# alvgaona/heart-sounds-segmentation

Hardware: AMD Instinct MI355X
Metric: PCG windows/sec FSST (1 kHz, 2000-sample) (higher is better)
Workload: dtype f32

## Files before the change

heart_sounds_segmentation_amd/csrc/fsst_canon128.hpp:

```cpp
#pragma once
#include "fsst_mfma128.hpp"

namespace hssfsst {

using h8 = _Float16 __attribute__((ext_vector_type(8)));
using u2 = unsigned __attribute__((ext_vector_type(2)));
using u4 = unsigned __attribute__((ext_vector_type(4)));
using lds_u2 = __attribute__((address_space(3))) u2;
using lds_u4 = __attribute__((address_space(3))) u4;

#define HSS_RARE_VMEM_DONE() __builtin_amdgcn_s_waitcnt(0x0f70)
constexpr int kCanonTileFrames = 64;
constexpr int kCanonRecs = 192;
constexpr int kCanonErrMul = 4;
constexpr int kCanonFlagWords = 8;
constexpr int kCanonTieWords = 32;

template <int KLO, int KC>
struct CanonCfg {
    static_assert(KC % 2 == 0 && KC >= 2 && KC <= 24 && KLO >= 0 && KLO + KC <= 32, "even band of <= 24 rows inside rows 0..31");
    static constexpr int NWIN = 128;
    static constexpr int KHI = KLO + KC - 1;
    static constexpr int H0 = KLO / 4, H1 = KHI / 4;
    static constexpr int COV0 = 4 * H0, COVN = 4 * (H1 - H0 + 1);
    static constexpr int LD = odd_up(COVN + 1), LDF = plane_ldf(KC), KOFF = KLO - COV0;
    static constexpr bool stored(int s, int half) { return 2 * s + half >= H0 && 2 * s + half <= H1; }
    static constexpr int need_row(int row)
    {
        int best = NWIN;
        for (int k = KLO; k <= KHI; ++k)
            for (int tw = 0; tw < 2; ++tw) {
                const int r = tw ? (NWIN - k) % NWIN : k;
                int d = row > r ? row - r : r - row;
                if (NWIN - d < d) d = NWIN - d;
                if (d < best) best = d;
            }
        return best;
    }
    static constexpr int need(int s, int half)
    {
        int best = NWIN;
        for (int r = 0; r < 4; ++r) {
            const int d = need_row(8 * s + 4 * half + r);
            if (d < best) best = d;
        }
        return best;
    }
    static constexpr float thr(int s, int half)
    {
        const int nd = need(s, half);
        return (nd <= 1 ? 0.5f : static_cast<float>(nd) - 0.5f) - static_cast<float>(1 + (nd <= 1 ? 0 : nd)) * kTieMargin;
    }
    static_assert(KLO >= 1, "row 0 is its own twin: acc_source / canon_put want the band above it");
    static constexpr int wave_floats() { return 2 * kCanonRecs + 2 * 16 * LD + kCanonFlagWords + kCanonTieWords; }
};


constexpr float kOffsetErr2 = 0.0625f;
struct CanonTile {
    float R2s;
    float inv;
    float r2s;
    float mean_s;
    __device__ __forceinline__ float eoff() const { return mean_s != 0.0f ? kOffsetErr2 : 0.0f; }
};

constexpr int kCanonYcGroup = 33;
constexpr int kCanonYcFrame = 4 * kCanonYcGroup * 2;
constexpr int kCanonYcRight = 80;
constexpr int kCanonZcFloats = kCanonYcFrame + 4 * 32 * 64 * 2 + 4 * 32 * kCanonYcRight * 2;
constexpr float kMeanTheta = 0.5f;

template <bool OFFS = true>
__device__ __forceinline__ CanonTile canon_land(const float (&sreg)[3], u2* xrec, float r2scale_s, float inv_c, int lane, int t0, int n)
{
    float e2 = 0.0f, s1 = 0.0f;
#pragma unroll
    for (int k = 0; k < 3; ++k) { e2 = fmaf(sreg[k], sreg[k], e2); s1 += sreg[k]; }
    const int inside = min(t0 + 128, n) - max(t0 - 64, 0);
    TileEnergy te = tile_energy(e2, s1, 0.0f);
    te.C = static_cast<float>(max(inside, 0));
    te.dcdom = te.E > 0.0f && te.S1 * te.S1 >= kDcTheta * te.C * te.E;
    auto stage = [&](const float (&x)[3], float Es, float E, float mean) -> CanonTile {
        const int eb = static_cast<int>((__float_as_uint(Es) >> 23) & 0xffu);
        const int hb = (eb - 127 + 2) >> 1;
        const int se = (eb == 0 || eb == 255) ? 127 : 127 + 14 - hb;
        const float sx = __uint_as_float(static_cast<unsigned>(se) << 23);
        CanonTile t;
        t.inv = __uint_as_float(static_cast<unsigned>(254 - se) << 23) * inv_c;
        t.R2s = r2scale_s * (E * sx) * sx;
        t.r2s = r2scale_s;
        t.mean_s = mean * sx;
#pragma unroll
        for (int k = 0; k < 3; ++k) {
            const float v = x[k] * sx;
            const _Float16 x1 = static_cast<_Float16>(v);
            const _Float16 x2 = static_cast<_Float16>(v - static_cast<float>(x1));
            const unsigned b1 = __builtin_bit_cast(unsigned short, x1), b2 = __builtin_bit_cast(unsigned short, x2);
            xrec[lane + 64 * k] = u2{b1 | (b1 << 16), b2 | (b2 << 16)};
        }
        wave_sync();
        return t;
    };
    if (__builtin_expect(te.E > 0.0f && te.S1 * te.S1 >= kMeanTheta * te.C * te.E, 0)) {
        if constexpr (!OFFS) { CanonTile r{}; r.mean_s = __builtin_nanf(""); return r; }
        const float mean = te.S1 / te.C;
        float x[3], ea = 0.0f;
#pragma unroll
        for (int k = 0; k < 3; ++k) {
            const int gi = t0 + lane + 64 * k - 64;
            x[k] = (gi >= 0 && gi < n) ? sreg[k] - mean : 0.0f;
            ea = fmaf(x[k], x[k], ea);
        }
        const float E = __int_as_float(__builtin_amdgcn_readfirstlane(__float_as_int(piece_sums(ea, 0.0f, 0.0f, 0.0f))));
        return stage(x, (E > 0.0f) ? E : te.S1 * mean, E, mean);
    }
    return stage(sreg, te.E, te.E, 0.0f);
}

struct CanonMove { int row; bool tie; };
__device__ __forceinline__ CanonMove canon_decide(int kpi, float num, float den, float R2, float eoff)
{
    constexpr int NWIN = 128;
    float shift = num * __builtin_amdgcn_rcpf(den);
    if (!(fabsf(shift) <= 1.0e6f)) shift = 0.0f;
    const float a = static_cast<float>(kpi) + shift;
    float fr = a - floorf(a) - 0.5f;
    const float s1 = 1.0f + fabsf(shift);
    asm volatile("" : "+v"(fr));
    CanonMove m;
    m.tie = fr * fr * den < (kTieErr2 * kCanonErrMul) * s1 * s1 * fmaf(eoff, den, R2) && den > kTieFloor2 * R2;
    const float r = truncf(a + copysignf(0.5f, a));
    m.row = static_cast<int>(r) & (NWIN - 1);
    return m;
}
template <int KLO, int KC, int S>
__device__ __forceinline__ bool canon_put(f2* row0, int kpi, int row, f2 V)
{
    constexpr int NWIN = 128;
    int t = row;
    float vy = V.y;
    if (!(static_cast<unsigned>(row - KLO) < static_cast<unsigned>(KC))) {
        if (!(row > NWIN / 2 && kpi != 0)) return false;
        t = NWIN - row; vy = -V.y;
        if (!(static_cast<unsigned>(t - KLO) < static_cast<unsigned>(KC))) return false;
    }
    if (S < 3 && (t >> 3) > S) return true;
    float* q = reinterpret_cast<float*>(row0 + t);
    __hip_atomic_fetch_add(q, V.x, __ATOMIC_RELAXED, __HIP_MEMORY_SCOPE_WORKGROUP);
    __hip_atomic_fetch_add(q + 1, vy, __ATOMIC_RELAXED, __HIP_MEMORY_SCOPE_WORKGROUP);
    return false;
}

template <int KLO, int KC, int TAPB = 4, bool OFFS = true, class XSig = const float*>
__device__ __forceinline__ void canon_group(const u2* xrec, const float* atab, f2* own_base, int* flag, int* tq,
                                            const double* wtab, const double* twtab, const CanonTile& tile, f2 tiny, int lane_o,
                                            XSig xsig, int n, int tg, const float* zc)
{
// ... 555 lines not shown
```

heart_sounds_segmentation_amd/csrc/fsst_launch_shape.hpp:

```cpp
#pragma once

#include <algorithm>
#include <cstddef>
#include <cstdint>
#include <vector>

namespace hssfsst {

constexpr int kMaxLdsBytes = 160 * 1024;
constexpr int kFpw128 = 64;
constexpr int kPartFloats = 8;

struct Core128Regions {
    int g0[3];
    int gpc[3];
    int npc[3];
};

inline Core128Regions core128_regions(int ngroups, long long nsig = -1)
{
    Core128Regions r{};
    const int tail2 = ngroups >= 32 ? 6 : 0;
    const int tail4 = ngroups >= 32 ? 16 : 0;
    if (ngroups < 32) {
// ... 84 lines not shown
    int rq = 0;
    bool fast = false;
    bool stripes03 = false;
    size_t lds_fixed = 0, lds_per_wave = 0;
};
constexpr MfmaFacts mfma_facts(int nwin, int klo, int K, bool stack)
{
    MfmaFacts f;
    f.fast = stack && (K & 1) == 0 && K <= 24;
    if (!mfma_length(nwin)) return f;
    const int nt = mfma_taps(nwin), rq = nwin / nt, min_waves = (nwin == 512) ? 2 : 4;
    const size_t fixed = (core128_atab_floats(rq, nt) + kCtlFloats) * sizeof(float);
    const size_t per_wave = static_cast<size_t>(wave_lds_floats(kFpw128, klo, K, rq, nt)) * sizeof(float);
    if (fixed + min_waves * per_wave > static_cast<size_t>(kMaxLdsBytes)) return f;
    f.nt = nt; f.rq = rq; f.lds_fixed = fixed; f.lds_per_wave = per_wave;
    f.stripes03 = own_s0(klo, rq) == 0 && own_s1(klo, K, rq) == 3;
    return f;
}
constexpr size_t core128_lds_bytes(const MfmaFacts& f, int wpb, bool pair)
{
    const size_t regions = pair ? wpb / 2 : wpb;
    return f.lds_fixed + regions * (f.lds_per_wave + (pair ? kPairFloats * sizeof(float) : 0));
}

struct Core128PlainRow { int nt, rq; bool fast; int wpb, s1c; bool pair; };
constexpr Core128PlainRow kCore128Plain[] = {
    {16, 8, true, 16, 3, false}, {16, 8, true, 16, -1, false},
    {16, 8, false, 16, -1, false}, {16, 8, false, 8, -1, false}, {16, 8, false, 4, -1, false},
    {16, 16, true, 8, -1, false}, {16, 16, false, 8, 3, false}, {16, 16, false, 8, -1, false},
    {16, 16, false, 4, -1, false}, {16, 16, true, 4, -1, false},
    {32, 16, true, 8, -1, true}, {32, 16, false, 8, -1, true}, {32, 16, false, 6, -1, true}, {32, 16, false, 4, -1, true},
    {32, 16, true, 8, -1, false}, {32, 16, false, 8, -1, false}, {32, 16, false, 6, -1, false}, {32, 16, true, 4, -1, false},
    {32, 16, false, 4, -1, false}, {32, 16, false, 3, -1, false}, {32, 16, false, 2, -1, false}, {32, 16, true, 2, -1, false},
};
constexpr int kCore128PlainRows = static_cast<int>(sizeof(kCore128Plain) / sizeof(kCore128Plain[0]));
constexpr int core128_plain_row(const MfmaFacts& f, bool no_pair)
{
    for (int i = 0; i < kCore128PlainRows; ++i) {
        const Core128PlainRow& r = kCore128Plain[i];
        if (r.nt == f.nt && r.rq == f.rq && r.fast == f.fast && (r.s1c < 0 || f.stripes03) && !(r.pair && no_pair)
            && core128_lds_bytes(f, r.wpb, r.pair) <= static_cast<size_t>(kMaxLdsBytes))
            return i;
    }
    return -1;
}

constexpr bool fused_rounds_full(int64_t batch, int64_t grid)
{
    const int64_t rounds = (batch + grid - 1) / grid;
    return !(batch < grid || rounds * grid * 100 > batch * 112);
}

constexpr int kT16MaxCpc = 8;
struct Team16Geometry {
    bool ok = false;
    int T = 0;
    int cpc_shift = 0;
    int nteams = 0, grid = 0;
    int slots = 0;
};
constexpr Team16Geometry team16_geometry(int G, int64_t batch, long long xstride, int cus, int WPB, int DEPTH, int pslots, int ms)
{
    Team16Geometry g;
    if (G < 1 || G > kFusedMaxGroups) return g;
    int T = 1;
    while ((WPB / 2) * T < G) T *= 2;
    if (T > cus || T > 64) return g;
    int cpc = 1, cpc_shift = 0;
    while (cpc * T < G) { cpc *= 2; ++cpc_shift; }
    if (cpc > WPB || cpc > kT16MaxCpc || G / T < 1) return g;
    if (cpc < 4 && T > 1) return g;
    int nteams = cus / T;
    if (batch < nteams) nteams = static_cast<int>(batch);
    if ((batch + nteams - 1) / nteams > 65535) return g;
    if (xstride < 1 || xstride > 0x7fffffffLL || batch > 0x7fffffffLL) return g;
    const int held_pos = WPB * (DEPTH + 3);
    const int lead = (held_pos + G / T - 1) / (G / T) + 1;
    int slots = 8;
    while (slots < 2 * lead + 2) slots *= 2;
    if (slots > ms) return g;
    if (lead + 1 > pslots) return g;
    g.ok = true; g.T = T; g.cpc_shift = cpc_shift; g.nteams = nteams; g.grid = nteams * T; g.slots = slots;
    return g;
}

struct ZscoreShape {
    int64_t grid;
    int slices;
    bool fused;
};
constexpr ZscoreShape zscore_shape(int64_t batch)
{
    int64_t zgrid = 4096;
    int slices = 1;
    if (batch < 1024) {
        slices = static_cast<int>(1024 / batch);
        if (slices > 32) slices = 32;
    }
    if (zgrid > batch * slices) zgrid = batch * slices;
    const bool fused = slices == 1 && zgrid == batch && batch >= 512;
    return {zgrid, slices, fused};
}

struct DftShape {
    int G;
    int waves;
    long long nitems;
    long long blocks;
};
constexpr DftShape dft_shape(int nk4, int K, int ncols, int64_t batch)
{
    int G = 1, best_waves = -1;
    for (int cand = 4; cand >= 1; cand >>= 1) {
        const size_t pw = static_cast<size_t>(dft_wave_lds_floats(nk4, K, cand)) * sizeof(float);
        int w = static_cast<int>(static_cast<size_t>(kMaxLdsBytes) / pw);
        if (w > 8) w = 8;
        if (w < 1) continue;
        int per_cu = static_cast<int>(static_cast<size_t>(kMaxLdsBytes) / (pw * w)) * w;
        if (per_cu > 32) per_cu = 32;
        if (per_cu >= 16) { G = cand; best_waves = per_cu; break; }
        if (per_cu > best_waves) { G = cand; best_waves = per_cu; }
    }
    if (ncols <= 16) G = 1;
    const size_t per_wave = static_cast<size_t>(dft_wave_lds_floats(nk4, K, G)) * sizeof(float);
    int waves = static_cast<int>(static_cast<size_t>(kMaxLdsBytes) / per_wave);
    if (waves > 8) waves = 8;
    if (waves < 1) return {G, 0, 0, 0};
    const int ntiles = (ncols + 16 * G - 1) / (16 * G);
    const long long nitems = static_cast<long long>(batch) * ntiles;
    long long blocks = (nitems + waves - 1) / waves;
    if (blocks > 256 * 64) blocks = 256 * 64;
    return {G, waves, nitems, blocks};
}

}
// ... 1 lines not shown
```

heart_sounds_segmentation_amd/csrc/fsst_team16.hpp:

```cpp
#pragma once
#include "fsst_mfma128.hpp"
#include "fsst_canon128.hpp"

namespace hssfsst {

using gu64 = __attribute__((address_space(1))) unsigned long long;

constexpr int kT16PartFloats = 6;
constexpr int kT16BlockWords = 8;
constexpr int kT16MaxBlocks = kFusedMaxGroups / kStatBlock;
constexpr int kT16SlotWords = kT16MaxBlocks * kT16BlockWords;
constexpr int kT16MaxSlots = 64;
constexpr int kT16StatFloats = 12;
constexpr int t16_ctl_base(int slots) { return 16 + 64 + 192 + 2 * slots + kT16StatFloats * slots; }
constexpr int t16_ctl_floats(int pslots, int slots) { return t16_ctl_base(slots) + pslots * (kT16MaxCpc * kT16PartFloats + 2); }
template <int KLO, int KC>
constexpr int t16_room() { return 160 * 1024 / 4 - kCanonLdsTabFloats - 16 * CanonCfg<KLO, KC>::wave_floats(); }
template <int KLO, int KC>
constexpr int t16_slots() { return t16_room<KLO, KC>() >= t16_ctl_floats(16, kT16MaxSlots) ? kT16MaxSlots : kT16MaxSlots / 2; }
template <int KLO, int KC>
constexpr int t16_pslots()
{
    constexpr int room = t16_room<KLO, KC>(), sl = t16_slots<KLO, KC>();
    return room >= t16_ctl_floats(32, sl) ? 32 : room >= t16_ctl_floats(16, sl) ? 16 : 0;
}

struct Team16Params {
    const float* x;
    float* out;
    const float* atab;
    const double* wtab;
    const double* twtab;
    unsigned long long* mail;
    unsigned* status;
    float r2scale_s;
    float inv_c;
    int n, nsig, col0, ncols;
    long long xstride;
    int team;
    int cpc_shift;
    int slots;
    unsigned seq;
    unsigned spin_ticks;
    unsigned* arrive;
    unsigned arrive_base;
    unsigned* abort_word;
    unsigned* fallbacks;
    unsigned launch;
    unsigned* done;
    unsigned done_base;
    unsigned* host_done;
    double inv_total, inv_total1;
};


constexpr int kT16HeldBase = 104;
#define HSS_T16_PAIRS(X) X(0, 104, 105) X(1, 106, 107) X(2, 108, 109) X(3, 110, 111) X(4, 112, 113) X(5, 114, 115) \
                         X(6, 116, 117) X(7, 118, 119) X(8, 120, 121) X(9, 122, 123) X(10, 124, 125) X(11, 126, 127)
template <int P>
__device__ __forceinline__ void held_put(f2 a, f2 b)
{
#define HSS_T16_PUT(N, LO, HI) if constexpr (P == N) asm volatile("v_pk_mul_f32 v[" #LO ":" #HI "], %0, %1" :: "v"(a), "v"(b) : "v" #LO, "v" #HI);
    HSS_T16_PAIRS(HSS_T16_PUT)
#undef HSS_T16_PUT
}
template <int P>
__device__ __forceinline__ f2 held_zscore(f2 m)
{
    f2 d, e;
#define HSS_T16_ZS(N, LO, HI) if constexpr (P == N) asm volatile("v_pk_add_f32 %0, v[" #LO ":" #HI "], %1 op_sel:[0,0] op_sel_hi:[1,0] neg_lo:[0,1] neg_hi:[0,1]" : "=v"(d) : "v"(m));
    HSS_T16_PAIRS(HSS_T16_ZS)
#undef HSS_T16_ZS
    asm("v_pk_mul_f32 %0, %1, %2 op_sel:[0,1] op_sel_hi:[1,1]" : "=v"(e) : "v"(d), "v"(m));
    return e;
}

template <class OT>
__device__ __forceinline__ void team16_store4(char* dst, f2 lo, f2 hi)
{
    static_assert(sizeof(OT) == 2, "2-byte output elements");
    using o2 = OT __attribute__((ext_vector_type(2)));
    using w2 = unsigned __attribute__((ext_vector_type(2)));
    const w2 w = {__builtin_bit_cast(unsigned, __builtin_convertvector(lo, o2)), __builtin_bit_cast(unsigned, __builtin_convertvector(hi, o2))};
    __builtin_nontemporal_store(w, reinterpret_cast<w2*>(dst));
}

template <int KLO, int KC, int WPB, int DEPTH, class OT = float>
__global__ __launch_bounds__(64 * WPB, WPB / 4) __attribute__((amdgpu_num_vgpr(52))) void fsst_team16_kernel(Team16Params p)
{
    constexpr int OB = static_cast<int>(sizeof(OT));
    using C = CanonCfg<KLO, KC>;
    static_assert(WPB % 4 == 0 && DEPTH >= 1 && DEPTH <= 2, "whole waves per SIMD; two held groups (v104 .. v127)");
    static_assert(DEPTH == 2, "the kernel is compiled for 104 allocatable registers + 24 fixed ones");
    constexpr int K = KC, ATAB = kCanonLdsTabFloats;
    extern __shared__ __attribute__((aligned(16))) float smem[];
    const int n = p.n;
    const int lane = threadIdx.x & 63;
    const int wv = __builtin_amdgcn_readfirstlane(threadIdx.x >> 6);
    float* atab = smem;
    int* next_q = reinterpret_cast<int*>(smem + ATAB);
    unsigned* dead = reinterpret_cast<unsigned*>(smem + ATAB) + 1;
    unsigned* cls_lds = reinterpret_cast<unsigned*>(smem + ATAB + 16);
    unsigned* ppk_lds = reinterpret_cast<unsigned*>(smem + ATAB + 80);
    unsigned* ready = reinterpret_cast<unsigned*>(smem + ATAB + 272);
    constexpr int MS = t16_slots<KLO, KC>(), PSLOTS = t16_pslots<KLO, KC>();
    unsigned* claim = ready + MS;
    float4* fin = reinterpret_cast<float4*>(smem + ATAB + 272 + 2 * MS);
    static_assert(PSLOTS >= 16, "the CU's own partials need LDS beside the wave regions");
    float* part_lds = smem + ATAB + t16_ctl_base(MS);
    int* pcnt_lds = reinterpret_cast<int*>(part_lds + PSLOTS * kT16MaxCpc * kT16PartFloats);
    float* wbase = smem + ATAB + t16_ctl_floats(PSLOTS, MS) + wv * C::wave_floats();
    u2* xrec = reinterpret_cast<u2*>(wbase);
    f2* own_base = reinterpret_cast<f2*>(wbase + 2 * kCanonRecs);
    int* flag = reinterpret_cast<int*>(own_base + 16 * C::LD);
    int* tq = flag + kCanonFlagWords;

    unsigned arrived = 0u;
    if (threadIdx.x == 64) arrived = __hip_atomic_fetch_add(p.arrive, 1u, __ATOMIC_RELAXED, __HIP_MEMORY_SCOPE_AGENT) - p.arrive_base;
    for (int i = threadIdx.x; i < ATAB; i += 64 * WPB) atab[i] = p.atab[i];
    if (lane < kCanonFlagWords) flag[lane] = 0;
    if (lane < kCanonTieWords) tq[lane] = 0;
    if (threadIdx.x < 16 && threadIdx.x != 2) next_q[threadIdx.x] = 0;
    for (int i = threadIdx.x; i < 2 * MS; i += 64 * WPB) ready[i] = 0u;
    if (threadIdx.x < 2 * PSLOTS) pcnt_lds[threadIdx.x] = 0;
    if (threadIdx.x == 64) next_q[2] = static_cast<int>(arrived);
    if (wv == 0) {
        unsigned cofs = 0u;
#pragma unroll
        for (int i = 0; i < 3; ++i) {
            const unsigned c = (4u * static_cast<unsigned>(lane + 64 * i)) % static_cast<unsigned>(2 * K);
            const unsigned nim = (c >= static_cast<unsigned>(K) ? 1u : 0u) + (c + 2 >= static_cast<unsigned>(K) ? 1u : 0u);
            cofs |= (16u * nim) << (8 * i);
            ppk_lds[i * 64 + lane] = canon_store_offsets<KLO, KC>(lane + 64 * i);
        }
        cls_lds[lane] = cofs;
    }
    __syncthreads();

    using kparams = const __attribute__((address_space(4))) Team16Params;
    kparams* const kp_ = (kparams*)__builtin_amdgcn_kernarg_segment_ptr();
    auto P = [&]() -> kparams* { kparams* q = kp_; asm volatile("" : "+s"(q)); return q; };

    auto aborted = [&]() -> bool {
        return __hip_atomic_load(P()->abort_word, __ATOMIC_RELAXED, __HIP_MEMORY_SCOPE_AGENT) == P()->launch;
    };
    auto gave_up = [&]() {
        if (lane == 0) {
            __hip_atomic_store(P()->abort_word, P()->launch, __ATOMIC_RELAXED, __HIP_MEMORY_SCOPE_AGENT);
            __hip_atomic_store((gu32*)(P()->fallbacks), P()->launch, __ATOMIC_RELAXED, __HIP_MEMORY_SCOPE_SYSTEM);
            __hip_atomic_store(dead, 1u, __ATOMIC_RELAXED, __HIP_MEMORY_SCOPE_WORKGROUP);
        }
    };
    auto is_dead = [&]() -> bool { return __hip_atomic_load(dead, __ATOMIC_RELAXED, __HIP_MEMORY_SCOPE_WORKGROUP) != 0u; };
    auto leave = [&]() { asm volatile("s_endpgm" ::: "memory"); };
    auto expired = [&](unsigned since) -> bool {
        return static_cast<unsigned>(wall_clock64()) - since > P()->spin_ticks || is_dead() || aborted();
    };

    const int virt = __builtin_amdgcn_readfirstlane(next_q[2]);
    if (static_cast<unsigned>(virt) >= gridDim.x) { gave_up(); return; }
    const unsigned abort_seen = __hip_atomic_load(P()->abort_word, __ATOMIC_RELAXED, __HIP_MEMORY_SCOPE_AGENT);
    const int T = p.team, cpcs = p.cpc_shift, cpc = 1 << cpcs;
    const int member = virt & (T - 1), team = virt / T;
    const int nteams = static_cast<int>(gridDim.x) / T;
    const int nk = (p.nsig > team) ? (p.nsig - team + nteams - 1) / nteams : 0;
    const int nwork = nk << cpcs;
    const int ncols = p.ncols, cend = p.col0 + p.ncols;
    const int G = (ncols + 15) >> 4;
    const int cg0 = p.col0 >> 4;
    const int smask = p.slots - 1;
    constexpr int nwords = kT16SlotWords;
    gu64* mail = (gu64*)(p.mail) + static_cast<size_t>(team) * static_cast<size_t>(p.slots) * nwords;
    const int nblocks = (G + kStatBlock - 1) / kStatBlock;
    const unsigned sig_bytes = static_cast<unsigned>(ncols) * (2 * K * OB);

    f2 tiny = {1.0e-37f, 0.0f};
    asm volatile("" : "+s"(tiny));
// ... 94 lines not shown
        int lane_r = lane;
        asm volatile("" : "+v"(lane_r));
        const unsigned t0 = static_cast<unsigned>(wall_clock64());
        for (unsigned spins = 0;; ++spins) {
            if ((spins & 15u) == 0u && try_claim(ko)) {
                resolve_owned(ko, t0, lane_r); return;
            }
            if ((spins & 31u) == 31u && expired(t0)) { gave_up(); leave(); }
            if (is_dead()) leave();
            __builtin_amdgcn_s_sleep(4);
            if (stats_ready(ko)) return;
        }
    };

    auto emit_held = [&](auto SL, int ko_h, int g_h) {
        constexpr int sl = decltype(SL)::value;
        int lane_r = lane;
        asm volatile("" : "+v"(lane_r));
        __builtin_amdgcn_fence(__ATOMIC_ACQUIRE, "workgroup");
        const unsigned cofs = cls_lds[lane_r];
        const char* tb = reinterpret_cast<const char*>(fin + 3 * (ko_h & smask));
        char* obase = reinterpret_cast<char*>(P()->out) + static_cast<unsigned long long>(static_cast<unsigned>(team + ko_h * nteams)) * sig_bytes +
                      static_cast<unsigned>(g_h * (16 * 2 * K * OB));
        const unsigned voff = static_cast<unsigned>(lane_r) * (4u * OB);
        const int nvalid = min(16, ncols - g_h * 16);
        auto put = [&](auto I) {
            constexpr int i = decltype(I)::value;
            const float4 tt = *reinterpret_cast<const float4*>(tb + ((cofs >> (8 * i)) & 0xffu));
            const f2 lo = held_zscore<6 * sl + 2 * i>(f2{tt.x, tt.y});
            const f2 hi = held_zscore<6 * sl + 2 * i + 1>(f2{tt.z, tt.w});
            if constexpr (OB == 4) __builtin_nontemporal_store(f4{lo.x, lo.y, hi.x, hi.y}, reinterpret_cast<f4*>(obase + (voff + 1024u * static_cast<unsigned>(i))));
            else team16_store4<OT>(obase + (voff + (256u * OB) * static_cast<unsigned>(i)), lo, hi);
        };
        if (__builtin_expect(nvalid == 16, 1)) {
            static_for<3>([&](auto I) {
                constexpr int i = decltype(I)::value;
                if constexpr (64 * (i + 1) <= 8 * K) put(I);
                else if constexpr (64 * i < 8 * K) { if (lane_r + 64 * i < 8 * K) put(I); }
            });
        } else {
            asm volatile("");
            const int lim = nvalid * (K >> 1);
            static_for<3>([&](auto I) { if (lane_r + 64 * decltype(I)::value < lim) put(I); });
        }
    };

    int nheld = 0;
    int ko_hs[DEPTH], g_hs[DEPTH];
#pragma unroll
    for (int d = 0; d < DEPTH; ++d) { ko_hs[d] = 0; g_hs[d] = 0; }

    bool c_valid = false;
    int ko = 0, g = 0;
    CanonTile tile{};
    auto land = [&]() {
        int lane_t = lane;
        asm volatile("" : "+v"(lane_t));
        tile = canon_land<true>(sreg, xrec, P()->r2scale_s, P()->inv_c, lane_t, ((g_d + cg0) & ~3) * 16, n);
        ko = ko_d; g = g_d; c_valid = true; d_valid = false;
    };
    int slot = 0;
    draw(-1);
    if (saw_dead || abort_seen == P()->launch) return;
    if (d_valid) { land(); draw(-1); }
    for (;;) {
        if (saw_dead) leave();
        if (!c_valid) {
            if (!d_valid) { draw(-1); if (saw_dead) leave(); }
            if (!d_valid) break;
            land();
        }
        int lane_o = lane;
        asm volatile("" : "+v"(lane_o));
        const unsigned b = static_cast<unsigned>(team + ko * nteams);
        const int tg = P()->col0 + g * 16;
        {
            const int lag = (d_valid ? ko_d : ko + 2) - ko;
            if (lag >= 2) __builtin_amdgcn_s_setprio(2); else if (lag == 1) __builtin_amdgcn_s_setprio(1); else __builtin_amdgcn_s_setprio(0);
        }
        canon_group<KLO, KC, 2, true>(xrec + ((g + cg0) & 3) * 16, atab, own_base, flag, tq, P()->wtab, P()->twtab, tile, tiny, lane_o,
                                           [&]() -> const float* { return P()->x + static_cast<unsigned long long>(b) * static_cast<unsigned>(P()->xstride); }, n, tg, P()->atab + kCanonAtabFloats);
        const float inv_cur = tile.inv;
        const int ko_cur = ko, g_cur = g;
        c_valid = false;
        HSS_RARE_VMEM_DONE();
        if (d_valid) land();
        {
            const int nvalid = min(16, cend - tg);
            f2 piv;
            const float w = canon_stats<KLO, KC>(own_base, nvalid, inv_cur, lane_o, piv);
            const int pos = g_cur & (cpc - 1);
            const int ps = ko_cur & (PSLOTS - 1);
            float* pe = part_lds + (ps * kT16MaxCpc + pos) * kT16PartFloats;
            const unsigned pa = static_cast<unsigned>(reinterpret_cast<size_t>((lds_float*)pe)) + (static_cast<unsigned>(lane_o) >> 4) * 4u;
            const unsigned pcnt_a = static_cast<unsigned>(reinterpret_cast<size_t>((__attribute__((address_space(3))) int*)(pcnt_lds + 2 * ps + (pos >> 2))));
            int before = 0;
            const bool known = ((q_last + 1) >> cpcs) > ko_cur;
            if (__builtin_expect(known, 1)) {
                const unsigned nq_a = static_cast<unsigned>(reinterpret_cast<size_t>((__attribute__((address_space(3))) int*)next_q));
                unsigned one = 1u, before_v, qi_v, dd_v;
                unsigned long long keep;
                asm volatile("s_mov_b64 %0, exec\n\ts_mov_b32 exec_lo, 0x00010001\n\ts_mov_b32 exec_hi, 0x00010001\n\tds_write_b32 %4, %5\n\t"
                             "s_mov_b64 exec, 1\n\tds_write_b64 %4, %6 offset:16\n\t"
                             "ds_add_rtn_u32 %1, %7, %9\n\tds_add_rtn_u32 %2, %8, %9\n\tds_read_b32 %3, %8 offset:4\n\t"
                             "s_mov_b64 exec, %0\n\ts_waitcnt lgkmcnt(0)"
                             : "=&s"(keep), "=&v"(before_v), "=&v"(qi_v), "=&v"(dd_v)
                             : "v"(pa), "v"(w), "v"(piv), "v"(pcnt_a), "v"(nq_a), "v"(one) : "memory");
                before = static_cast<int>(before_v);
                ask_qi = static_cast<int>(qi_v);
                ask_dd = dd_v;
                wave_sync();
            } else {
                unsigned long long keep;
                asm volatile("s_mov_b64 %0, exec\n\ts_mov_b32 exec_lo, 0x00010001\n\ts_mov_b32 exec_hi, 0x00010001\n\tds_write_b32 %1, %2\n\t"
                             "s_mov_b64 exec, 1\n\tds_write_b64 %1, %3 offset:16\n\ts_mov_b64 exec, %0"
                             : "=&s"(keep) : "v"(pa), "v"(w), "v"(piv) : "memory");
                wave_sync();
                if (lane == 0) before = __hip_atomic_fetch_add(pcnt_lds + 2 * ps + (pos >> 2), 1, __ATOMIC_RELAXED, __HIP_MEMORY_SCOPE_WORKGROUP);
                draw_ask(ko_cur);
            }
            const int blk = g_cur >> 2, bfirst = blk << 2;
            const int expect = min(kStatBlock, G - bfirst);
            if (__builtin_amdgcn_readfirstlane(before) + 1 == expect) {
                __builtin_amdgcn_s_setprio(3);
                if (lane == 0) __hip_atomic_store(pcnt_lds + 2 * ps + (pos >> 2), 0, __ATOMIC_RELAXED, __HIP_MEMORY_SCOPE_WORKGROUP);
                wave_sync();
                int lane_b = lane;
                asm volatile("" : "+v"(lane_b));
                const int q = lane_b & 3, h = q >> 1, pc = (lane_b >> 2) & 3;
                const float* pb = part_lds + (ps * kT16MaxCpc + (pos & ~3) + pc) * kT16PartFloats;
                const double cnt = static_cast<double>(min(16, ncols - 16 * (bfirst + pc))) * static_cast<double>(K);
                const double mom = piece_moment(q, static_cast<double>(pb[2 * h]), static_cast<double>(pb[2 * h + 1]), static_cast<double>(pb[4 + h]), cnt);
                auto from_row = [&](int ctrl) -> double {
// ... 115 lines not shown
```

heart_sounds_segmentation_amd/csrc/hssfsst.hip:

```cpp
#include "../../include/hssfsst.h"

#include <hip/hip_runtime.h>

#include <algorithm>
#include <cmath>
#include <cstdarg>
#include <cstdio>
#include <cstring>
#include <chrono>
#include <mutex>
#include <dlfcn.h>
#include <cstdlib>
#include <array>
#include <atomic>
#include <memory>
#include <new>
#include <thread>
#include <vector>
#include <type_traits>
#include <utility>

#include "fsst_kernels.hpp"
#include "fsst_mfma128.hpp"
#include "fsst_canon128.hpp"
// ... 454 lines not shown
    cp.status = pl->d_status;
    name_kernel(cx.kernel, WPB, grid, "fsst_core128_kernel<%d, %d, %d, %s, %d, %d, true>", NT, RQ, kFpw128, FAST ? "true" : "false", WPB, S1C);
    hipLaunchKernelGGL(kern, dim3(static_cast<unsigned>(grid)), dim3(64 * WPB), lds, cx.st, cp);
    HIP_TRY(hipGetLastError());
    return 1;
}

int ensure_status(hssfsst_plan* pl)
{
    if (pl->d_status) return 0;
    void* h = nullptr;
    HIP_TRY(hipHostMalloc(&h, sizeof(unsigned), hipHostMallocMapped));
    *static_cast<volatile unsigned*>(h) = 0u;
    void* d = nullptr;
    HIP_TRY(hipHostGetDevicePointer(&d, h, 0));
    pl->h_status = static_cast<volatile unsigned*>(h);
    pl->d_status = static_cast<unsigned*>(d);
    return 0;
}

int ensure_team_words(hssfsst_plan* pl, hipStream_t st)
{
    if (pl->d_arrive.get()) return 0;
    if (int rc = pl->d_arrive.grow(4)) return rc;
    HIP_TRY(hipMemsetAsync(pl->d_arrive.get(), 0, 4 * sizeof(unsigned), st));
    pl->arrive_total = 0;
    pl->done_total = 0;
    void* h = nullptr;
    HIP_TRY(hipHostMalloc(&h, 4 * sizeof(unsigned), hipHostMallocMapped));
    for (int i = 0; i < 4; ++i) static_cast<volatile unsigned*>(h)[i] = 0u;
    void* d = nullptr;
    HIP_TRY(hipHostGetDevicePointer(&d, h, 0));
    pl->h_fallback = static_cast<volatile unsigned*>(h);
    pl->d_fallback = static_cast<unsigned*>(d);
    return 0;
}

template <int KLO, int KC, int WPB, int DEPTH, class OT>
constexpr auto team16_kernel()
{
    return &hssfsst::fsst_team16_kernel<KLO, KC, WPB, DEPTH, OT>;
}
template <class OT>
constexpr const char* out_type_suffix() { return sizeof(OT) == 4 ? "" : std::is_same<OT, _Float16>::value ? ", f16" : ", bf16"; }

template <int KLO, int KC, int WPB, int DEPTH, class OT = float>
int launch_team16(hssfsst_plan* pl, ExecCtx& cx, const hssfsst::Core128Params& cp, int64_t batch, int ngroups, void* hout = nullptr)
{
    using namespace hssfsst;
    hipStream_t st = cx.st;
    if constexpr (sizeof(OT) == 2) {
        if (hout == nullptr || (reinterpret_cast<uintptr_t>(hout) & 7) != 0) return 0;
    }
    constexpr int PSLOTS = t16_pslots<KLO, KC>();
    constexpr int MS = t16_slots<KLO, KC>();
    size_t lds = canon_lds_bytes(t16_ctl_floats(PSLOTS, MS), CanonCfg<KLO, KC>::wave_floats(), WPB);
    if (lds > static_cast<size_t>(kMaxLdsBytes)) return 0;
    if (lds < 84 * 1024) lds = 84 * 1024;
    auto kern = team16_kernel<KLO, KC, WPB, DEPTH, OT>();
    static std::atomic<unsigned long long> lds_ok{0};
    if (int rc = allow_full_lds(kern, pl->device, lds_ok)) return rc;
    if (int rc = resident_blocks(pl, pl->team16_cus, kern, 64 * WPB, lds, true)) return rc;
    if (pl->team16_cus < 1) return 0;
    const Team16Geometry geo = team16_geometry(ngroups, batch, cp.xstride, pl->team16_cus, WPB, DEPTH, PSLOTS, MS);
    if (!geo.ok) return 0;
    const int T = geo.T, nteams = geo.nteams, grid = geo.grid, slots = geo.slots;
    int rc;
    if ((rc = ensure_status(pl)) != 0) return rc;
    const size_t words = static_cast<size_t>(nteams) * slots * kT16SlotWords;
    if (words > pl->d_mail.cap) {
        if ((rc = pl->d_mail.grow(words)) != 0) return rc;
        HIP_TRY(hipMemsetAsync(pl->d_mail.get(), 0, pl->d_mail.cap * sizeof(unsigned long long), st));
        pl->team_seq = 0;
    }
    if (++pl->team_seq > 0xffffu) {
        HIP_TRY(hipMemsetAsync(pl->d_mail.get(), 0, pl->d_mail.cap * sizeof(unsigned long long), st));
        pl->team_seq = 1;
    }
    Team16Params tp{};
    tp.x = cp.x; tp.out = sizeof(OT) == 4 ? cp.out : static_cast<float*>(hout); tp.atab = pl->d_atab16.get(); tp.wtab = cp.wtab; tp.twtab = cp.twtab;
    tp.mail = pl->d_mail.get(); tp.status = pl->d_status; tp.r2scale_s = pl->canon_r2s; tp.inv_c = pl->canon_inv_c;
    tp.n = cp.n; tp.nsig = cp.nsig; tp.col0 = cp.col0; tp.ncols = cp.ncols; tp.xstride = cp.xstride;
    tp.team = T; tp.cpc_shift = geo.cpc_shift; tp.slots = slots; tp.seq = pl->team_seq;
    {
        const double total = static_cast<double>(KC) * static_cast<double>(cp.ncols);
        tp.inv_total = 1.0 / total; tp.inv_total1 = 1.0 / (total - 1.0);
    }
    tp.spin_ticks = 500u * 100u;
    if ((rc = ensure_team_words(pl, st)) != 0) return rc;
    if (++pl->team_launch == 0u) pl->team_launch = 1u;
    tp.abort_word = pl->d_arrive.get() + 1; tp.fallbacks = pl->d_fallback; tp.launch = pl->team_launch;
    const bool force_fallback = debug_switches().team_force_fallback;
    if (force_fallback) {
        HIP_TRY(hipMemcpyAsync(pl->d_arrive.get() + 1, &pl->team_launch, sizeof(unsigned), hipMemcpyHostToDevice, st));
        HIP_TRY(hipMemcpyAsync(pl->d_fallback, &pl->team_launch, sizeof(unsigned), hipMemcpyHostToDevice, st));
    }
    tp.arrive = pl->d_arrive.get(); tp.arrive_base = pl->arrive_total;
    pl->arrive_total += static_cast<unsigned>(grid);
    if (cx.want_done_word && !force_fallback) {
        tp.done = pl->d_arrive.get() + 2; tp.done_base = pl->done_total; tp.host_done = pl->d_fallback + 2;
        pl->done_total += static_cast<unsigned>(grid);
        cx.flagged_launch = pl->team_launch;
    }
    name_kernel(cx.kernel, WPB, grid, "fsst_team16_kernel<%d, %d, %d, %d%s> teams of %d", KLO, KC, WPB, DEPTH, out_type_suffix<OT>(), T);
    hipLaunchKernelGGL(kern, dim3(static_cast<unsigned>(grid)), dim3(64 * WPB), lds, st, tp);
    HIP_TRY(hipGetLastError());
    cx.team_launch = pl->team_launch;
    return 1;
}

constexpr int kCanonBands[][2] = {{4, 22}, {2, 24}};

bool plan_is_canon(const hssfsst_plan* pl) { return pl->canon_idx >= 0; }
template <class F>
int canon_dispatch(const hssfsst_plan* pl, F&& f)
{
    switch (pl->canon_idx) {
    case 0: return f(std::integral_constant<int, kCanonBands[0][0]>{}, std::integral_constant<int, kCanonBands[0][1]>{});
    case 1: return f(std::integral_constant<int, kCanonBands[1][0]>{}, std::integral_constant<int, kCanonBands[1][1]>{});
    default: return fail(HSSFSST_EINVAL, "canon_dispatch: not a canonical-class plan");
    }
}

hssfsst::CanonParams canon_params(const hssfsst_plan* pl, const ExecCtx& cx, const hssfsst::Core128Params& cp)
{
    hssfsst::CanonParams q{};
    q.x = cp.x; q.out = cp.out; q.partials = cp.partials; q.atab = pl->d_atab16.get(); q.wtab = cp.wtab; q.twtab = cp.twtab;
    q.r2scale_s = pl->canon_r2s; q.inv_c = pl->canon_inv_c;
    q.n = cp.n; q.mode = cp.mode; q.nsig = cp.nsig; q.col0 = cp.col0; q.ncols = cp.ncols; q.xstride = cp.xstride; q.reg = cp.reg;
    q.status = cp.status;
    q.gate = cx.gate; q.gate_val = cx.gate_val;
    return q;
}

template <int KLO, int KC, bool RAGGED = false>
int launch_canon_band(hssfsst_plan* pl, ExecCtx& cx, const hssfsst::Core128Params& cp, int64_t nchunks)
// ... 2114 lines not shown
```

Before: 5.957 million.

## Share landed tile records across waves via an LDS ring in team16 kernel

Replaces each wave's private copy of the canonicalised tile records with a block-shared LDS ring. Slots are keyed by signal and tile and carry a tag, so a wave that finds the tile already landed by a sibling wave reads the stored CanonTile instead of recomputing the energy and split-f16 records. This is meant to remove redundant canon_land work and per-wave record storage, at the cost of an LDS tag check, extra geometry constraints, and a dynamic LDS size that may change occupancy or disable the path.

New measurement: 6.063 million, median of 6. Within noise of the previous version (+1.8%).

```diff
diff --git a/heart_sounds_segmentation_amd/csrc/fsst_canon128.hpp b/heart_sounds_segmentation_amd/csrc/fsst_canon128.hpp
--- a/heart_sounds_segmentation_amd/csrc/fsst_canon128.hpp
+++ b/heart_sounds_segmentation_amd/csrc/fsst_canon128.hpp
@@ -71,7 +71,6 @@
 constexpr int kCanonZcFloats = kCanonYcFrame + 4 * 32 * 64 * 2 + 4 * 32 * kCanonYcRight * 2;
 constexpr float kMeanTheta = 0.5f;
 
-template <bool OFFS = true>
 __device__ __forceinline__ CanonTile canon_land(const float (&sreg)[3], u2* xrec, float r2scale_s, float inv_c, int lane, int t0, int n)
 {
     float e2 = 0.0f, s1 = 0.0f;
@@ -103,7 +102,6 @@
         return t;
     };
     if (__builtin_expect(te.E > 0.0f && te.S1 * te.S1 >= kMeanTheta * te.C * te.E, 0)) {
-        if constexpr (!OFFS) { CanonTile r{}; r.mean_s = __builtin_nanf(""); return r; }
         const float mean = te.S1 / te.C;
         float x[3], ea = 0.0f;
 #pragma unroll
diff --git a/heart_sounds_segmentation_amd/csrc/fsst_launch_shape.hpp b/heart_sounds_segmentation_amd/csrc/fsst_launch_shape.hpp
--- a/heart_sounds_segmentation_amd/csrc/fsst_launch_shape.hpp
+++ b/heart_sounds_segmentation_amd/csrc/fsst_launch_shape.hpp
@@ -160,14 +160,56 @@
 }
 
 constexpr int kT16MaxCpc = 8;
+constexpr int kT16PartFloats = 6;
+constexpr int kT16MaxSlots = 64;
+constexpr int kT16StatFloats = 12;
+constexpr int t16_ctl_base(int slots) { return 16 + 64 + 192 + 2 * slots + kT16StatFloats * slots; }
+constexpr int t16_ctl_floats(int pslots, int slots) { return t16_ctl_base(slots) + pslots * (kT16MaxCpc * kT16PartFloats + 2); }
+constexpr int canon_own_ld(int klo, int K) { return odd_up(4 * ((klo + K - 1) / 4 - klo / 4 + 1) + 1); }
+constexpr int t16_wave_floats(int klo, int K) { return 2 * 16 * canon_own_ld(klo, K) + 8 + 32; }
+constexpr int kT16RingRecFloats = 2 * 192;
+constexpr int kT16RingTileAt = kT16RingRecFloats, kT16RingTagAt = kT16RingRecFloats + 4;
+constexpr int kT16RingSlotFloats = kT16RingRecFloats + 8;
+struct Team16Lds {
+    int ms = 0, pslots = 0;
+    int ctl_floats = 0, wave_floats = 0;
+    int ring_room = 0;
+};
+constexpr Team16Lds team16_lds(int klo, int K, int wpb = 16)
+{
+    Team16Lds l;
+    l.wave_floats = t16_wave_floats(klo, K);
+    const int room = kMaxLdsBytes / 4 - kCanonLdsTabFloats - wpb * l.wave_floats;
+    l.ms = room >= t16_ctl_floats(16, kT16MaxSlots) ? kT16MaxSlots : kT16MaxSlots / 2;
+    l.pslots = room >= t16_ctl_floats(32, l.ms) ? 32 : room >= t16_ctl_floats(16, l.ms) ? 16 : 0;
+    l.ctl_floats = t16_ctl_floats(l.pslots, l.ms);
+    l.ring_room = room - l.ctl_floats;
+    return l;
+}
+
 struct Team16Geometry {
     bool ok = false;
     int T = 0;
     int cpc_shift = 0;
     int nteams = 0, grid = 0;
     int slots = 0;
-};
-constexpr Team16Geometry team16_geometry(int G, int64_t batch, long long xstride, int cus, int WPB, int DEPTH, int pslots, int ms)
+    int lead = 0;
+    int ring_sig = 0, ring_tiles = 0;
+};
+constexpr uint32_t team16_ring_magic(int ring_sig) { return static_cast<uint32_t>(((1ull << 32) + ring_sig - 1) / ring_sig); }
+constexpr int team16_ring_slot(int ko, int g, int cg0, int cpc_shift, int ring_sig, int ring_tiles, uint32_t magic)
+{
+    const int first = g & ~((1 << cpc_shift) - 1);
+    const int turn = static_cast<int>((static_cast<uint64_t>(static_cast<uint32_t>(ko)) * magic) >> 32);
+    return (ko - turn * ring_sig) * ring_tiles + (((g + cg0) >> 2) - ((first + cg0) >> 2));
+}
+constexpr size_t team16_lds_bytes(const Team16Lds& l, int wpb, const Team16Geometry& g)
+{
+    return (static_cast<size_t>(kCanonLdsTabFloats) + l.ctl_floats + static_cast<size_t>(wpb) * l.wave_floats +
+            static_cast<size_t>(g.ring_sig) * g.ring_tiles * kT16RingSlotFloats) * sizeof(float);
+}
+constexpr Team16Geometry team16_geometry(int G, int64_t batch, long long xstride, int cus, int WPB, int DEPTH, int pslots, int ms,
+                                         int cg0 = 0, int ring_room = kMaxLdsBytes / 4)
 {
     Team16Geometry g;
     if (G < 1 || G > kFusedMaxGroups) return g;
@@ -188,7 +230,11 @@
     while (slots < 2 * lead + 2) slots *= 2;
     if (slots > ms) return g;
     if (lead + 1 > pslots) return g;
+    const int ring_sig = lead + 1;
+    const int ring_tiles = (((cg0 & 3) + cpc - 1) >> 2) + 1;
+    if (ring_sig > 64 || static_cast<long long>(ring_sig) * ring_tiles * kT16RingSlotFloats > ring_room) return g;
     g.ok = true; g.T = T; g.cpc_shift = cpc_shift; g.nteams = nteams; g.grid = nteams * T; g.slots = slots;
+    g.lead = lead; g.ring_sig = ring_sig; g.ring_tiles = ring_tiles;
     return g;
 }
 
diff --git a/heart_sounds_segmentation_amd/csrc/fsst_team16.hpp b/heart_sounds_segmentation_amd/csrc/fsst_team16.hpp
--- a/heart_sounds_segmentation_amd/csrc/fsst_team16.hpp
+++ b/heart_sounds_segmentation_amd/csrc/fsst_team16.hpp
@@ -6,24 +6,14 @@
 
 using gu64 = __attribute__((address_space(1))) unsigned long long;
 
-constexpr int kT16PartFloats = 6;
 constexpr int kT16BlockWords = 8;
 constexpr int kT16MaxBlocks = kFusedMaxGroups / kStatBlock;
 constexpr int kT16SlotWords = kT16MaxBlocks * kT16BlockWords;
-constexpr int kT16MaxSlots = 64;
-constexpr int kT16StatFloats = 12;
-constexpr int t16_ctl_base(int slots) { return 16 + 64 + 192 + 2 * slots + kT16StatFloats * slots; }
-constexpr int t16_ctl_floats(int pslots, int slots) { return t16_ctl_base(slots) + pslots * (kT16MaxCpc * kT16PartFloats + 2); }
+static_assert(kT16RingRecFloats == 2 * kCanonRecs && kT16RingTileAt % 4 == 0 && kT16RingSlotFloats % 4 == 0, "a ring slot: the tile's records, then its CanonTile on a 16-byte line");
 template <int KLO, int KC>
-constexpr int t16_room() { return 160 * 1024 / 4 - kCanonLdsTabFloats - 16 * CanonCfg<KLO, KC>::wave_floats(); }
+constexpr int t16_slots() { return team16_lds(KLO, KC).ms; }
 template <int KLO, int KC>
-constexpr int t16_slots() { return t16_room<KLO, KC>() >= t16_ctl_floats(16, kT16MaxSlots) ? kT16MaxSlots : kT16MaxSlots / 2; }
-template <int KLO, int KC>
-constexpr int t16_pslots()
-{
-    constexpr int room = t16_room<KLO, KC>(), sl = t16_slots<KLO, KC>();
-    return room >= t16_ctl_floats(32, sl) ? 32 : room >= t16_ctl_floats(16, sl) ? 16 : 0;
-}
+constexpr int t16_pslots() { return team16_lds(KLO, KC).pslots; }
 
 struct Team16Params {
     const float* x;
@@ -40,6 +30,9 @@
     int team;
     int cpc_shift;
     int slots;
+    int ring_sig;
+    int ring_tiles;
+    unsigned ring_magic;
     unsigned seq;
     unsigned spin_ticks;
     unsigned* arrive;
@@ -109,9 +102,11 @@
     static_assert(PSLOTS >= 16, "the CU's own partials need LDS beside the wave regions");
     float* part_lds = smem + ATAB + t16_ctl_base(MS);
     int* pcnt_lds = reinterpret_cast<int*>(part_lds + PSLOTS * kT16MaxCpc * kT16PartFloats);
-    float* wbase = smem + ATAB + t16_ctl_floats(PSLOTS, MS) + wv * C::wave_floats();
-    u2* xrec = reinterpret_cast<u2*>(wbase);
-    f2* own_base = reinterpret_cast<f2*>(wbase + 2 * kCanonRecs);
+    constexpr int WF = t16_wave_floats(KLO, KC);
+    static_assert(WF == C::wave_floats() - 2 * kCanonRecs, "a wave's region: CanonCfg's without the tile's records");
+    float* wbase = smem + ATAB + t16_ctl_floats(PSLOTS, MS) + wv * WF;
+    f2* own_base = reinterpret_cast<f2*>(wbase);
+    float* ring = smem + ATAB + t16_ctl_floats(PSLOTS, MS) + WPB * WF;
     int* flag = reinterpret_cast<int*>(own_base + 16 * C::LD);
     int* tq = flag + kCanonFlagWords;
 
@@ -123,6 +118,7 @@
     if (threadIdx.x < 16 && threadIdx.x != 2) next_q[threadIdx.x] = 0;
     for (int i = threadIdx.x; i < 2 * MS; i += 64 * WPB) ready[i] = 0u;
     if (threadIdx.x < 2 * PSLOTS) pcnt_lds[threadIdx.x] = 0;
+    for (int i = threadIdx.x; i < p.ring_sig * p.ring_tiles; i += 64 * WPB) ring[i * kT16RingSlotFloats + kT16RingTagAt] = 0.0f;
     if (threadIdx.x == 64) next_q[2] = static_cast<int>(arrived);
     if (wv == 0) {
         unsigned cofs = 0u;
@@ -323,11 +319,32 @@
 
     bool c_valid = false;
     int ko = 0, g = 0;
+    int rec_at = 0;
     CanonTile tile{};
+    static_assert((ATAB + t16_ctl_floats(PSLOTS, MS) + WPB * WF) % 4 == 0, "ring slots on 16-byte lines");
     auto land = [&]() {
         int lane_t = lane;
         asm volatile("" : "+v"(lane_t));
-        tile = canon_land<true>(sreg, xrec, P()->r2scale_s, P()->inv_c, lane_t, ((g_d + cg0) & ~3) * 16, n);
+        const int at = ATAB + t16_ctl_floats(PSLOTS, MS) + WPB * WF + team16_ring_slot(ko_d, g_d, cg0, cpcs, p.ring_sig, p.ring_tiles, p.ring_magic) * kT16RingSlotFloats;
+        float* sl = smem + at;
+        const unsigned sa = static_cast<unsigned>(reinterpret_cast<size_t>((lds_float*)sl));
+        const unsigned want = static_cast<unsigned>(ko_d) + 1u;
+        unsigned tag;
+        f4 tf;
+        asm volatile("ds_read_b32 %0, %2 offset:%3\n\tds_read_b128 %1, %2 offset:%4\n\ts_waitcnt lgkmcnt(0)"
+                     : "=&v"(tag), "=&v"(tf) : "v"(sa), "n"(4 * kT16RingTagAt), "n"(4 * kT16RingTileAt) : "memory");
+        if (static_cast<unsigned>(__builtin_amdgcn_readfirstlane(static_cast<int>(tag))) == want) {
+            auto first = [](float v) -> float { return __int_as_float(__builtin_amdgcn_readfirstlane(__float_as_int(v))); };
+            tile.R2s = first(tf.x); tile.inv = first(tf.y); tile.r2s = first(tf.z); tile.mean_s = first(tf.w);
+        } else {
+            tile = canon_land(sreg, reinterpret_cast<u2*>(sl), P()->r2scale_s, P()->inv_c, lane_t, ((g_d + cg0) & ~3) * 16, n);
+            const f4 tv = {tile.R2s, tile.inv, tile.r2s, tile.mean_s};
+            unsigned long long keep;
+            asm volatile("s_mov_b64 %0, exec\n\ts_mov_b64 exec, 1\n\tds_write_b128 %1, %2 offset:%5\n\tds_write_b32 %1, %3 offset:%4\n\ts_mov_b64 exec, %0"
+                         : "=&s"(keep) : "v"(sa), "v"(tv), "v"(want), "n"(4 * kT16RingTagAt), "n"(4 * kT16RingTileAt) : "memory");
+            wave_sync();
+        }
+        rec_at = at;
         ko = ko_d; g = g_d; c_valid = true; d_valid = false;
     };
     int slot = 0;
@@ -349,7 +366,7 @@
             const int lag = (d_valid ? ko_d : ko + 2) - ko;
             if (lag >= 2) __builtin_amdgcn_s_setprio(2); else if (lag == 1) __builtin_amdgcn_s_setprio(1); else __builtin_amdgcn_s_setprio(0);
         }
-        canon_group<KLO, KC, 2, true>(xrec + ((g + cg0) & 3) * 16, atab, own_base, flag, tq, P()->wtab, P()->twtab, tile, tiny, lane_o,
+        canon_group<KLO, KC, 2, true>(reinterpret_cast<const u2*>(smem + rec_at) + ((g + cg0) & 3) * 16, atab, own_base, flag, tq, P()->wtab, P()->twtab, tile, tiny, lane_o,
                                            [&]() -> const float* { return P()->x + static_cast<unsigned long long>(b) * static_cast<unsigned>(P()->xstride); }, n, tg, P()->atab + kCanonAtabFloats);
         const float inv_cur = tile.inv;
         const int ko_cur = ko, g_cur = g;
diff --git a/heart_sounds_segmentation_amd/csrc/hssfsst.hip b/heart_sounds_segmentation_amd/csrc/hssfsst.hip
--- a/heart_sounds_segmentation_amd/csrc/hssfsst.hip
+++ b/heart_sounds_segmentation_amd/csrc/hssfsst.hip
@@ -530,18 +530,18 @@
     if constexpr (sizeof(OT) == 2) {
         if (hout == nullptr || (reinterpret_cast<uintptr_t>(hout) & 7) != 0) return 0;
     }
-    constexpr int PSLOTS = t16_pslots<KLO, KC>();
-    constexpr int MS = t16_slots<KLO, KC>();
-    size_t lds = canon_lds_bytes(t16_ctl_floats(PSLOTS, MS), CanonCfg<KLO, KC>::wave_floats(), WPB);
-    if (lds > static_cast<size_t>(kMaxLdsBytes)) return 0;
-    if (lds < 84 * 1024) lds = 84 * 1024;
+    constexpr Team16Lds L = team16_lds(KLO, KC, WPB);
+    constexpr int PSLOTS = L.pslots, MS = L.ms;
+    if (L.pslots < 16 || L.ring_room < 1) return 0;
     auto kern = team16_kernel<KLO, KC, WPB, DEPTH, OT>();
     static std::atomic<unsigned long long> lds_ok{0};
     if (int rc = allow_full_lds(kern, pl->device, lds_ok)) return rc;
-    if (int rc = resident_blocks(pl, pl->team16_cus, kern, 64 * WPB, lds, true)) return rc;
+    if (int rc = resident_blocks(pl, pl->team16_cus, kern, 64 * WPB, 84 * 1024, true)) return rc;
     if (pl->team16_cus < 1) return 0;
-    const Team16Geometry geo = team16_geometry(ngroups, batch, cp.xstride, pl->team16_cus, WPB, DEPTH, PSLOTS, MS);
+    const Team16Geometry geo = team16_geometry(ngroups, batch, cp.xstride, pl->team16_cus, WPB, DEPTH, PSLOTS, MS, cp.col0 >> 4, L.ring_room);
     if (!geo.ok) return 0;
+    size_t lds = team16_lds_bytes(L, WPB, geo);
+    if (lds < 84 * 1024) lds = 84 * 1024;
     const int T = geo.T, nteams = geo.nteams, grid = geo.grid, slots = geo.slots;
     int rc;
     if ((rc = ensure_status(pl)) != 0) return rc;
@@ -559,7 +559,7 @@
     tp.x = cp.x; tp.out = sizeof(OT) == 4 ? cp.out : static_cast<float*>(hout); tp.atab = pl->d_atab16.get(); tp.wtab = cp.wtab; tp.twtab = cp.twtab;
     tp.mail = pl->d_mail.get(); tp.status = pl->d_status; tp.r2scale_s = pl->canon_r2s; tp.inv_c = pl->canon_inv_c;
     tp.n = cp.n; tp.nsig = cp.nsig; tp.col0 = cp.col0; tp.ncols = cp.ncols; tp.xstride = cp.xstride;
-    tp.team = T; tp.cpc_shift = geo.cpc_shift; tp.slots = slots; tp.seq = pl->team_seq;
+    tp.team = T; tp.cpc_shift = geo.cpc_shift; tp.slots = slots; tp.ring_sig = geo.ring_sig; tp.ring_tiles = geo.ring_tiles; tp.ring_magic = team16_ring_magic(geo.ring_sig); tp.seq = pl->team_seq;
     {
         const double total = static_cast<double>(KC) * static_cast<double>(cp.ncols);
         tp.inv_total = 1.0 / total; tp.inv_total1 = 1.0 / (total - 1.0);
```
